# cvjena/semantic-embeddings

Hardware: AMD Instinct MI355X
Metric: retrieval_Mpairs_per_sec (higher is better)
Workload: dtype f32

## Files before the change

### semantic-embeddings_amd/csrc/rank_rows.hip

```cpp
#include "se_common.h"
#include <stdlib.h>
#include <atomic>
#include <type_traits>

namespace se {

constexpr int RK_THREADS = 512;
constexpr int RK_WAVES = RK_THREADS / WAVE;
constexpr int RK_ITEMS = 16;
constexpr int RK_TILE = RK_THREADS * RK_ITEMS;
constexpr int RK_WCHUNK = RK_TILE / RK_WAVES;
constexpr int RK_NB = 256;

struct RankLds {
    uint32_t gbase[4][RK_NB];
    uint32_t wcnt[RK_WAVES][RK_NB];
    uint32_t tile_start[RK_NB];
    uint32_t wave_tot[RK_WAVES];
    uint32_t tkeys[RK_TILE];
    uint32_t tidx[RK_TILE];
};

__device__ __forceinline__ uint32_t wave_excl_scan(uint32_t v, uint32_t &total)
{
// ... 478 lines not shown
        const int first_pad_ = ((NROW) - wave_s * (ITEMS * WAVE)) >> 6;    \
        if (first_pad_ >= ITEMS - RR_PADS) {                                                                          \
            _Pragma("unroll") for (int s = ITEMS - RR_PADS; s < ITEMS; s++) { BODY }                                  \
        } else {                                                                                                      \
            _Pragma("unroll") for (int s = 0; s < ITEMS; s++) { BODY }                                                \
        }                                                                                                             \
    }
#define RR_IDX_SCATTER_IMG(AFTER_STORE)                                                                               \
    {                                                                                                                 \
        opaque(ir[0]);                                                                                                \
        uint32_t a_ = rr_dst_mad(ir[0], xb);                                                                          \
        _Pragma("unroll") for (int s = 0; s < ITEMS; s++) {                                                           \
            uint32_t an_ = 0;                                                                                         \
            if (s + 1 < ITEMS) { opaque(ir[s + 1]); an_ = rr_dst_mad(ir[s + 1], xb); }                                \
            lds_st16_hi(a_, ir[s]);                                                                        \
            AFTER_STORE                                                                                               \
            a_ = an_;                                                                                                 \
        }                                                                                                             \
    }
    if ((int64_t)blockIdx.x < Q) {
        const float *drow = row_ptr(blockIdx.x);
        const int n0 = row_len(blockIdx.x);
        int wpos = wpos0;
        opaque(wpos);
#pragma unroll
        for (int s = 0; s < ITEMS; s++) RR_LOAD_ONE(drow, wpos, s, n0)
        if constexpr (!RAWKEYS) RR_CANON(n0)
    }
    uint32_t pf_sink = 0;
    [[maybe_unused]] int img_level = 0;
    [[maybe_unused]] bool img_again = false;
    [[maybe_unused]] int img_skip0 = 0, img_pen0 = 0, img_skip1 = 0, img_pen1 = 0;
    for (int64_t row = blockIdx.x; row < Q;) {
        const bool more = row + gridDim.x < Q;
        [[maybe_unused]] const int n_next = row_len(more ? row + gridDim.x : row);
        constexpr bool SKIP_WAVES = HWORD && ITEMS <= 88;
        const bool wave_live = !SKIP_WAVES || wave * (ITEMS * WAVE) < row_len(row);
        constexpr bool LOAD_IN_SCATTER = IMG && !SKIP_WAVES;
        bool two = false;
        [[maybe_unused]] int n_out = 0;
        if constexpr (IMG) {
            const int n_row = row_len(row);
            if (!img_again) {
                if (img_skip1 > 0) { img_level = 2; img_skip1--; }
                else if (img_skip0 > 0) { img_level = 1; img_skip0--; }
                else img_level = 0;
            }
            bool attempt = img_level < 2;
            uint32_t cbits = 0, base = 0;
            if (attempt) {
                uint32_t mb = 0;
#pragma unroll
                for (int s = 0; s + 1 < ITEMS; s += 2) mb = max(max(mb, key[s] & 0x7FFFFFFFu), key[s + 1] & 0x7FFFFFFFu);
                if constexpr (ITEMS & 1) mb = max(mb, key[ITEMS - 1] & 0x7FFFFFFFu);
#pragma unroll
                for (int off = 32; off > 0; off >>= 1) mb = max(mb, (uint32_t)__shfl_xor((int)mb, off, 64));
                if (lane == 0) wave_tot[wave] = mb;
                static_assert(!IMG || (RR_IMG_SET_WORDS == 4 * RR_THREADS && RR_IMG_SET_WORDS == RR_WIDE_WORDS && RR_IMG_SET_WORDS <= RR_IMG_WL), "one uint4 per thread, inside the worklist");
                *reinterpret_cast<uint4 *>(wlist + 4 * tid) = make_uint4(0u, 0u, 0u, 0u);
                wg_barrier();
                if (tid == 0) { ictl[0] = 0; ictl[1] = 0; }
#pragma unroll
                for (int w = 0; w < RR_WAVES; w++) mb = max(mb, wave_tot[w]);
                mb = (uint32_t)__builtin_amdgcn_readfirstlane((int)mb);
                const uint32_t e = (mb >> 23) + ((mb & 0x7FFFFFu) > 0x400000u ? 1u : 0u) - (img_level == 0 ? 1u : 0u);
                two = mb >= 0x0D800000u && mb < 0x7E800000u;
                cbits = (e + 1u) << 23;
                base = e << 23;
            }
            if (two) {
                const float c = __uint_as_float(cbits);
                int wpos_ = wpos0;
                opaque(wpos_);
                const uint32_t pk_ = ((RR_IMG_NAN_PADHI + ((uint32_t)wpos_ & 15u)) << 20) | (((uint32_t)wpos_ & 63u) << 14);
                const uint32_t tb = lds_off(tagb) + (uint32_t)wpos_;
#pragma unroll
                for (int s = 0; s < ITEMS; s++) {
                    const uint32_t t = __float_as_uint(__uint_as_float(key[s]) + c);
                    const uint32_t q = (uint32_t)rr_clamp_i32(__builtin_elementwise_sub_sat((int32_t)t, (int32_t)base), 0, 0xFEFFFF);
                    asm volatile("ds_write_b8 %0, %1 offset:%2" ::"v"(tb), "v"(q), "n"(s * WAVE) : "memory");
                    key[s] = q << 8;
                }
                if (wave_s * (ITEMS * WAVE) + ITEMS * WAVE > n_row) {
                    RR_PAD_LOOP(n_row, key[s] = (wpos_ + s * WAVE >= n_row) ? pk_ : key[s];)
                }
            } else {
                RR_CANON(n_row)
            }
            RR_T(8)
        }
        if constexpr (WIDE && VAR == 2) {
            uint32_t *stat = wave_tot;
            uint2 *outl = reinterpret_cast<uint2 *>(wcnt);
            const int n_row = row_len(row);
            int32_t mxi = 0;
            uint32_t umx = 0;
#pragma unroll
            for (int s = 0; s + 1 < ITEMS; s += 2) {
                mxi = max(max(mxi, rr_clamp_i32((int32_t)key[s], 0, 0x7F800000)), rr_clamp_i32((int32_t)key[s + 1], 0, 0x7F800000));
                umx = max(max(umx, key[s]), key[s + 1]);
            }
            if constexpr (ITEMS & 1) { mxi = max(mxi, rr_clamp_i32((int32_t)key[ITEMS - 1], 0, 0x7F800000)); umx = max(umx, key[ITEMS - 1]); }
            mxi = umx > 0xFF800000u ? 0x7F800000 : mxi;
#pragma unroll
            for (int off = 32; off > 0; off >>= 1) mxi = max(mxi, __shfl_xor(mxi, off, 64));
            if (lane == 0) stat[wave] = (uint32_t)mxi;
            if (tid == 0) stat[2 * RR_WAVES] = 0;
            RR_T(9)
            wg_barrier();
            RR_T(10)
#pragma unroll
            for (int w = 0; w < RR_WAVES; w++) mxi = max(mxi, (int32_t)stat[w]);
            const int32_t kmax = __builtin_amdgcn_readfirstlane(mxi);
            const int32_t lo = kmax > (int32_t)RR_TWO_SPAN ? kmax - (int32_t)RR_TWO_SPAN : 1, lo1 = lo - 1;
            uint32_t below_l = 0;
            {
                int wpos = wpos0;
                opaque(wpos);
#pragma unroll
                for (int s = 0; s < ITEMS; s++) below_l += ((int32_t)key[s] < lo) ? 1u : 0u;
                if (wave_s * (ITEMS * WAVE) + ITEMS * WAVE > n_row) {
                    int32_t lo_b = lo;
                    opaque(lo_b);
                    RR_PAD_LOOP(n_row, below_l -= (wpos + s * WAVE >= n_row && (int32_t)key[s] < lo_b) ? 1u : 0u;)
                }
            }
            uint32_t below_w = below_l;
#pragma unroll
            for (int off = 32; off > 0; off >>= 1) below_w += (uint32_t)__shfl_xor((int)below_w, off, 64);
            if (lane == 0) stat[RR_WAVES + wave] = below_w;
            RR_T(11)
            wg_barrier();
            uint32_t below = 0;
#pragma unroll
            for (int w = 0; w < RR_WAVES; w++) below += stat[RR_WAVES + w];
            two = kmax > 0 && below <= (uint32_t)RR_TWO_OUT;
            n_out = (int)below;
            if (two) {
                int wpos = wpos0;
                opaque(wpos);
                if (below_w != 0) {
                    int32_t lo_c = lo;
                    opaque(lo_c);
#pragma unroll
                    for (int s = 0; s < ITEMS; s++)
                        if ((int32_t)key[s] < lo_c && wpos + s * WAVE < n_row)
                            outl[atomicAdd(&stat[2 * RR_WAVES], 1u)] = make_uint2(rr_key(key[s], false, 0u), (uint32_t)(wpos + s * WAVE));
                }
#pragma unroll
                for (int s = 0; s < ITEMS; s++)
                    key[s] = (uint32_t)rr_clamp_i32(__builtin_elementwise_sub_sat((int32_t)key[s], lo1), 0, 0xFFFFFF) << 8;
                if (wave_s * (ITEMS * WAVE) + ITEMS * WAVE > n_row) {
                    RR_PAD_LOOP(n_row, key[s] = (wpos + s * WAVE >= n_row) ? 0xFFFFFF00u : key[s];)
                }
            } else {
                RR_CANON(n_row)
            }
            RR_T(8)
        }
        __builtin_amdgcn_sched_barrier(0);
        {
            int wpos = wpos0;
            opaque(wpos);
#pragma unroll
            for (int s = 0; s < ITEMS; s++) ir[s] = (uint32_t)(wpos + s * WAVE) << 16;
        }
#pragma unroll 1
        for (int p = 0; p < NPASS; p++) {
            const int shift = two ? 8 + 12 * p : (WIDE ? p * 10 : p * BITS);
            const int end = two ? (p == 1 ? 32 : 20)
                                : (WIDE ? (p == 2 ? 32 : shift + 10) : ((shift + BITS < 32) ? shift + BITS : 32));
            const bool wide = WIDE && (two || p == 2);
            uint32_t *pcnt = wcnt;
            int pcw = CNT_WORDS;
            const bool shared0 = IMG && two && p == 0;
            if (shared0) {
                pcnt = wlist;
                pcw = 0;
            } else if (wide) {
                if (!(RAWKEYS && two && p == 0)) wg_barrier();
                pcnt = reinterpret_cast<uint32_t *>(xbuf);
                pcw = RR_WIDE_WORDS;
            }
            uint32_t *mycnt = pcnt + wave * pcw;
            const uint32_t cb = lds_off(mycnt);
            auto one_set = [&]() -> bool {
                if constexpr (!IMG) return false;
                int z = pcw;
                asm volatile("" : "+s"(z));
                return z == 0;
            };
            if constexpr (IMG) {
                if (!one_set()) {
#pragma unroll
                    for (int j = 0; j < CNT_WORDS / (4 * WAVE); j++) reinterpret_cast<uint4 *>(mycnt)[j * WAVE + lane] = make_uint4(0u, 0u, 0u, 0u);
                    if (wide) {
#pragma unroll
                        for (int j = CNT_WORDS / (4 * WAVE); j < RR_WIDE_WORDS / (4 * WAVE); j++) reinterpret_cast<uint4 *>(mycnt)[j * WAVE + lane] = make_uint4(0u, 0u, 0u, 0u);
                    }
                }
            } else {
#pragma unroll
                for (int j = 0; j < CNT_WORDS / WAVE; j++) mycnt[j * WAVE + lane] = 0;
                if (wide) {
#pragma unroll
                    for (int j = CNT_WORDS / WAVE; j < RR_WIDE_WORDS / WAVE; j++) mycnt[j * WAVE + lane] = 0;
                }
            }
            [[maybe_unused]] const uint32_t wlo = wide ? 11u : 10u, whi = (uint32_t)(end - shift) - wlo, hshift = (uint32_t)(shift + (int)wlo) & 31u;
            if constexpr (HWORD) {
                if (wave_live) {
                    uint32_t hr[RR_GH], hs[RR_GH], hg[RR_GH];
                    RRRankHW<ITEMS, PEEL>::run(ir, key, hr, hs, hg, (uint32_t)shift, hshift, wlo, whi, cb, lane, end >= 32 && !two);
                }
            }
            else RRRank<ITEMS>::run(ir, key, shift, lane, cb);
            lds_wait();
            RR_T(1)
            wg_barrier();
            if constexpr (!HWORD) {
            uint32_t ex = 0;
            if (tid < RK_NB) {
                uint32_t run = 0;
#pragma unroll
                for (int w = 0; w < RR_WAVES; w++) run += wcnt[w * RK_NB + tid];
                uint32_t wtot;
                ex = wave_excl_scan(run, wtot);
                if (lane == 63) wave_tot[wave] = wtot;
            }
            wg_barrier();
            if (tid < RK_NB) {
                for (int w = 0; w < wave; w++) ex += wave_tot[w];
#pragma unroll
                for (int w = 0; w < RR_WAVES; w++) {
                    const uint32_t c = wcnt[w * RK_NB + tid];
                    wcnt[w * RK_NB + tid] = ex;
                    ex += c;
                }
            }
            } else {
                const bool scanner = tid < RR_SCAN_THREADS;
                const int st = scanner ? tid : 0;
                uint32_t T0 = 0, T1 = 0, U0 = 0, U1 = 0;
#pragma unroll
                for (int w = 0; w < RR_WAVES; w++) {
                    if (w == 1 && one_set()) break;
                    const uint2 v = *reinterpret_cast<const uint2 *>(pcnt + w * pcw + 2 * st);
                    T0 += v.x; T1 += v.y;
                }
                if (wide) {
                    __builtin_amdgcn_sched_barrier(0);
#pragma unroll
                    for (int w = 0; w < RR_WAVES; w++) {
                        if (w == 1 && one_set()) break;
                        const uint2 v = *reinterpret_cast<const uint2 *>(pcnt + w * pcw + CNT_WORDS + 2 * st);
                        U0 += v.x; U1 += v.y;
                    }
                    __builtin_amdgcn_sched_barrier(0);
                }
                uint32_t wtot, wtot2 = 0, ex2 = 0;
                uint32_t ex = wave_excl_scan(T0 + T1, wtot);
                if (wide) ex2 = wave_excl_scan(U0 + U1, wtot2);
                if (scanner && lane == 63) { wave_tot[wave] = wtot; wave_tot[RR_SCAN_WAVES + wave] = wtot2; }
                wg_barrier();
                uint32_t all = 0, all2 = 0;
#pragma unroll
                for (int w = 0; w < RR_SCAN_WAVES; w++) {
                    const uint32_t wt = wave_tot[w], wt2 = wave_tot[RR_SCAN_WAVES + w];
                    all += wt; all2 += wt2;
                    ex += (w < wave) ? wt : 0u;
                    ex2 += (w < wave) ? wt2 : 0u;
                }
                ex2 += all;
                const uint32_t hi = (all + all2) << 16;
                ex += hi; ex2 += hi;
                if (scanner) {
                uint32_t s0 = ex, s1 = ex + T0;
#pragma unroll
                for (int w = 0; w < RR_WAVES; w++) {
                    if (w == 1 && one_set()) break;
                    uint2 *wp = reinterpret_cast<uint2 *>(pcnt + w * pcw + 2 * tid);
                    const uint2 v = *wp;
                    *wp = make_uint2(s0, s1);
                    s0 += v.x; s1 += v.y;
                }
                if (wide) {
                    __builtin_amdgcn_sched_barrier(0);
                    s0 = ex2; s1 = ex2 + U0;
#pragma unroll
                    for (int w = 0; w < RR_WAVES; w++) {
                        if (w == 1 && one_set()) break;
                        uint2 *wp = reinterpret_cast<uint2 *>(pcnt + w * pcw + CNT_WORDS + 2 * tid);
                        const uint2 v = *wp;
                        *wp = make_uint2(s0, s1);
                        s0 += v.x; s1 += v.y;
                    }
                }
                }
            }
            wg_barrier();
            RR_T(2)
            if (!(IMG && two)) { RR_PREFETCH_NEXT_ROW() }
            if (wave_live) {
#pragma unroll
            for (int s0 = 0; s0 < ITEMS; s0 += 8) {
                uint32_t first[8];
#pragma unroll
                for (int g = 0; g < 8; g++)
                    if (s0 + g < ITEMS) {
                        if constexpr (HWORD) first[g] = reinterpret_cast<const uint16_t *>(mycnt)[(__builtin_amdgcn_ubfe(key[s0 + g], (uint32_t)shift, wlo) << 1) | __builtin_amdgcn_ubfe(key[s0 + g], hshift, whi)];
                        else first[g] = mycnt[(key[s0 + g] >> shift) & 0xFFu];
                    }
#pragma unroll
                for (int g = 0; g < 8; g++)
                    if (s0 + g < ITEMS) {
                        ir[s0 + g] += first[g];
                        opaque(ir[s0 + g]);
                    }
                __builtin_amdgcn_sched_barrier(0);
            }
            }
            if (wide && !one_set()) wg_barrier();
            RR_T(3)
            if constexpr (LOAD_IN_SCATTER) {
                if (end >= 32) break;
            }
            if (wave_live) {
                if constexpr (LOAD_IN_SCATTER) {
                    RR_IDX_SCATTER_IMG()
                } else {
#pragma unroll
                    for (int s = 0; s < ITEMS; s++) { opaque(ir[s]); lds_st16_hi(RR_DST(ir[s]), ir[s]); }
                }
            }
            lds_wait();
            wg_barrier();
            RR_T(4)
            const bool last = end >= 32;
            if (last) {
                if constexpr (!SEG) break;
                else {
                    RR_STREAM_PLANE(0, row)
                    wg_barrier();
                }
            } else {
                if (wave_live) rr_read_back<ITEMS, true>(ir, ring, rt, rb);
                lds_wait();
                wg_barrier();
            }
            RR_T(5)
            if (wave_live) {
#pragma unroll
                for (int s = 0; s < ITEMS; s++) { opaque(ir[s]); lds_st16_hi(RR_DST(ir[s]), key[s]); }
            }
            lds_wait();
            wg_barrier();
            if (SEG && last) {
                RR_STREAM_PLANE(1, row)
            } else {
                if (wave_live) rr_read_back<ITEMS, true>(key, ring, rt, rb);
                lds_wait();
            }
            if (end < 16 || SEG) {
                wg_barrier();
                if (wave_live) {
#pragma unroll
                    for (int s = 0; s < ITEMS; s++) { opaque(ir[s]); lds_st16_lo(RR_DST(ir[s]), key[s]); }
                }
                lds_wait();
                wg_barrier();
                if (SEG && last) break;
                if (wave_live) rr_read_back<ITEMS, false>(key, ring, rt, rb);
                lds_wait();
            }
            RR_T(6)
        }
#undef RR_DST
        if constexpr (WIDE && VAR == 2) {
            if (two && n_out > 1) {
                const uint2 *outl = reinterpret_cast<const uint2 *>(wcnt);
                if (tid < n_out) {
                    const uint2 me = outl[tid];
                    int r = 0;
                    for (int j = 0; j < n_out; j++) {
                        const uint2 o = outl[j];
                        r += (o.x < me.x || (o.x == me.x && o.y < me.y)) ? 1 : 0;
                    }
                    xbuf[r] = (uint16_t)me.y;
                }
                wg_barrier();
            }
        }
        [[maybe_unused]] bool img_fail = false;
        if constexpr (IMG) {
            const float *drow = row_ptr(more ? row + gridDim.x : row);
            int wpos = wpos0;
            opaque(wpos);
            if constexpr (LOAD_IN_SCATTER) {
                RR_IDX_SCATTER_IMG(RR_LOAD_ONE(drow, wpos, s, n_next))
                lds_wait();
                wg_barrier();
                RR_T(4)
            } else {
#pragma unroll
                for (int s = 0; s < ITEMS; s++) RR_LOAD_ONE(drow, wpos, s, n_next)
            }
        }
        if constexpr (IMG) {
            if (two) {
                int n_row = row_len(row);
                int tsc = wave_s * WAVE + (int)wave_prefix_count(~0u, ~0u);
                opaque(n_row);
                opaque(tsc);
                const float *drow_cur = row_ptr(row);
                constexpr int NS = RR_THREADS * ITEMS;
                constexpr int NG = (NS / 8 + RR_THREADS - 1) / RR_THREADS;
                uint32_t S[NG];
                uint32_t nstart = 0;
                uint4 xg[NG];
                uint32_t nxg[NG];
#pragma unroll
                for (int g = 0; g < NG; g++) {
                    const int b0 = (tsc + RR_THREADS * g) * 8;
                    const int bs = b0 < NS ? b0 : 0;
                    xg[g] = *reinterpret_cast<const uint4 *>(xbuf + bs);
                    nxg[g] = xbuf[(tsc & 63) == 63 ? (bs + 8 < NS ? bs + 8 : bs) : 0];
                }
                constexpr int TD = 1;
                uint32_t t[TD + 1][9];
                auto tag_reads = [&](int g, uint32_t (&tt)[9]) {
                    const uint32_t xi[4] = {xg[g].x, xg[g].y, xg[g].z, xg[g].w};
#pragma unroll
                    for (int j = 0; j < 4; j++) {
                        tt[2 * j] = tagb[xi[j] & 0xFFFFu];
                        tt[2 * j + 1] = tagb[xi[j] >> 16];
                    }
                    tt[8] = tagb[nxg[g]];
                };
#pragma unroll
                for (int g = 0; g < TD && g < NG; g++) tag_reads(g, t[g % (TD + 1)]);
#pragma unroll
                for (int g = 0; g < NG; g++) {
                    if (g + TD < NG) tag_reads(g + TD, t[(g + TD) % (TD + 1)]);
                    const uint32_t (&tc)[9] = t[g % (TD + 1)];
                    const bool live = (tsc + RR_THREADS * g) * 8 < n_row - 1;
                    const uint32_t A = tc[0] | (tc[1] << 8) | (tc[2] << 16) | (tc[3] << 24), B = tc[4] | (tc[5] << 8) | (tc[6] << 16) | (tc[7] << 24);
                    const uint32_t t8 = (uint32_t)__builtin_amdgcn_update_dpp((int)tc[8], (int)tc[0], 0x130, 0xF, 0xF, false);
                    const uint32_t zA = A ^ __builtin_amdgcn_alignbyte(B, A, 1), zB = B ^ __builtin_amdgcn_alignbyte(t8, B, 1);
                    const uint32_t uA = (zA & 0x7F7F7F7Fu) + 0x7F7F7F7Fu, uB = (zB & 0x7F7F7F7Fu) + 0x7F7F7F7Fu;
                    const uint32_t eA = __builtin_amdgcn_bitop3_b32(uA, zA, 0x80808080u, 0x02), eB = __builtin_amdgcn_bitop3_b32(uB, zB, 0x80808080u, 0x02);
                    S[g] = live ? ((eA >> 7) | (eB >> 3)) : 0u;
                    nstart += (uint32_t)__popc(S[g]);
                }
                uint32_t slot = 0;
                {
                    const uint32_t ca = lds_off(&ictl[0]);
                    asm volatile("ds_add_rtn_u32 %0, %1, %2\n\ts_waitcnt lgkmcnt(0)" : "=v"(slot) : "v"(ca), "v"(nstart) : "memory");
                }
#pragma unroll
                for (int g = 0; g < NG; g++) {
                    uint32_t st = S[g];
                    const int b0 = (tsc + RR_THREADS * g) * 8;
                    while (st) {
                        const int bit = __builtin_ctz(st);
                        st &= st - 1u;
                        const int pos = b0 + (bit & 4) + (bit >> 3);
                        if (slot < (uint32_t)RR_IMG_WL) wlist[slot] = pos < n_row - 1 ? (uint32_t)pos : 0xFFFFFFFFu;
                        slot++;
                    }
                }
                if constexpr (PROF) { RR_T(9) }
                wg_barrier();
                const uint32_t nwork = ictl[0];
                img_fail = nwork > (uint32_t)RR_IMG_WL;
                RR_T(11)
                if (!img_fail) {
                    constexpr int GB = 2;
#pragma unroll 1
                    for (uint32_t e0 = 0; e0 < nwork; e0 += RR_THREADS * GB) {
                        uint32_t pp[GB], im[GB], ia[GB], ib[GB], ic[GB], id[GB], tm[GB], t0[GB], t2[GB], t3[GB], ka[GB], kb[GB], kc[GB];
#pragma unroll
                        for (int k = 0; k < GB; k++) {
                            const uint32_t e = e0 + (uint32_t)(k * RR_THREADS + tsc);
                            pp[k] = e < nwork ? wlist[e] : 0xFFFFFFFFu;
                        }
#pragma unroll
                        for (int k = 0; k < GB; k++) {
                            const uint32_t p = pp[k] != 0xFFFFFFFFu ? pp[k] : 0u;
                            im[k] = xbuf[p ? p - 1u : 0u]; ia[k] = xbuf[p]; ib[k] = xbuf[p + 1];
                            ic[k] = xbuf[p + 2 < (uint32_t)NS ? p + 2 : p]; id[k] = xbuf[p + 3 < (uint32_t)NS ? p + 3 : p];
                        }
#pragma unroll
                        for (int k = 0; k < GB; k++) { tm[k] = tagb[im[k]]; t0[k] = tagb[ia[k]]; t2[k] = tagb[ic[k]]; t3[k] = tagb[id[k]]; }
#pragma unroll
                        for (int k = 0; k < GB; k++) {
                            const bool mine = pp[k] != 0xFFFFFFFFu && !(pp[k] != 0u && tm[k] == t0[k]);
                            const bool three = mine && (int)pp[k] + 2 < n_row && t2[k] == t0[k];
                            ka[k] = kb[k] = kc[k] = 0u;
                            if (mine) {
                                ka[k] = __float_as_uint(drow_cur[ia[k]]);
                                kb[k] = __float_as_uint(drow_cur[ib[k]]);
                            }
                            if (three) kc[k] = __float_as_uint(drow_cur[ic[k]]);
                        }
                        uint32_t rare = 0;
#pragma unroll
                        for (int k = 0; k < GB; k++) {
                            if (pp[k] == 0xFFFFFFFFu) continue;
                            const uint32_t p = pp[k];
                            if (p != 0u && tm[k] == t0[k]) continue;
                            const bool three = (int)p + 2 < n_row && t2[k] == t0[k];
                            const bool more4 = three && (int)p + 3 < n_row && t3[k] == t0[k];
                            const uint64_t ca = ((uint64_t)rr_key(ka[k], false, 0u) << 32) | ia[k], cb = ((uint64_t)rr_key(kb[k], false, 0u) << 32) | ib[k],
                                           cc = ((uint64_t)rr_key(kc[k], false, 0u) << 32) | ic[k];
                            if (!three) {
                                if (ca > cb) { xbuf[p] = (uint16_t)ib[k]; xbuf[p + 1] = (uint16_t)ia[k]; }
                            } else if (!more4) {
                                const uint32_t ab = ca < cb, ac = ca < cc, bc = cb < cc;
                                const uint32_t ra = 2u - ab - ac, rb = ab + 1u - bc, rc = ac + bc;
                                if (ra != 0u || rb != 1u) {
                                    xbuf[p + ra] = (uint16_t)ia[k]; xbuf[p + rb] = (uint16_t)ib[k]; xbuf[p + rc] = (uint16_t)ic[k];
                                }
                            } else rare |= 1u << k;
                        }
                        static_assert(GB == 2, "the entry is picked by one select");
#pragma unroll 1
                        for (uint32_t k = 0; k < (uint32_t)GB; k++) {
                            if (!((rare >> k) & 1u)) continue;
                            const uint32_t p = k ? pp[1] : pp[0], tg = k ? t0[1] : t0[0];
                            int len = 4;
                            while (len <= RR_IMG_RUN && (int)p + len < n_row && tagb[xbuf[p + len]] == tg) len++;
                            if (len > RR_IMG_RUN) { ictl[1] = 1u; continue; }
                            uint32_t idx[RR_IMG_RUN];
                            uint64_t kk[RR_IMG_RUN];
#pragma unroll
                            for (int j = 0; j < RR_IMG_RUN; j++) idx[j] = xbuf[p + (uint32_t)(j < len ? j : 0)];
#pragma unroll
                            for (int j = 0; j < RR_IMG_RUN; j++) kk[j] = ((uint64_t)rr_key(__float_as_uint(drow_cur[idx[j]]), false, 0u) << 32) | idx[j];
#pragma unroll
                            for (int j = 0; j < RR_IMG_RUN; j++) {
                                uint32_t r = 0;
#pragma unroll
                                for (int i = 0; i < RR_IMG_RUN; i++)
                                    if (i != j) r += (i < len && kk[i] < kk[j]) ? 1u : 0u;
                                if (j < len) xbuf[p + r] = (uint16_t)idx[j];
                            }
                        }
                    }
                    wg_barrier();
                    img_fail = ictl[1] != 0u;
                }
                RR_T(10)
            }
        }
        if (!IMG || img_fail) {
            const float *drow = row_ptr((IMG && img_fail) ? row : (more ? row + gridDim.x : row));
            int wpos = wpos0;
            opaque(wpos);
#pragma unroll
            for (int s = 0; s < ITEMS; s++) RR_LOAD_ONE(drow, wpos, s, n_next)
        }
        if constexpr (IMG) {
#pragma unroll
            for (int s = 0; s < ITEMS; s++) opaque(key[s]);
            asm volatile("s_waitcnt vmcnt(0)" : "+v"(pf_sink) : : "memory");
        }
        int wt = tid;
        opaque(wt);
        const bool write_out = !IMG || !img_fail;
        if constexpr (SEG) {
            RR_STREAM_PLANE(2, row)
        } else if (!write_out) {
        } else if (idx64 == 2) {
            uint16_t *o = (uint16_t *)rank + row * ldr;
            _Pragma("unroll 2") for (int j = wt * 8; j < N; j += RR_THREADS * 8) {
                if (vec_ok && j + 7 < N) {
                    const rr_i32x4 v = *reinterpret_cast<const rr_i32x4 *>(xbuf + j);
                    __builtin_nontemporal_store(v, reinterpret_cast<rr_i32x4 *>(o + j));
                } else {
                    for (int e = 0; e < 8 && j + e < N; e++) o[j + e] = xbuf[j + e];
                }
            }
        } else if (idx64) {
            int64_t *o = (int64_t *)rank + row * ldr;
            uint2 nv = *reinterpret_cast<const uint2 *>(xbuf + (wt * 4 < N ? wt * 4 : 0));
            _Pragma("unroll 1") for (int j = wt * 4; j < N; j += RR_THREADS * 4) {
                const uint2 v = nv;
                const int jn = j + RR_THREADS * 4;
                nv = *reinterpret_cast<const uint2 *>(xbuf + (jn < N ? jn : 0));
                const int64_t e0 = v.x & 0xFFFFu, e1 = v.x >> 16, e2 = v.y & 0xFFFFu, e3 = v.y >> 16;
                if (vec_ok && j + 3 < N) {
                    __builtin_nontemporal_store((rr_i64x2){e0, e1}, reinterpret_cast<rr_i64x2 *>(o + j));
                    __builtin_nontemporal_store((rr_i64x2){e2, e3}, reinterpret_cast<rr_i64x2 *>(o + j + 2));
                } else {
                    o[j] = e0;
                    if (j + 1 < N) o[j + 1] = e1;
                    if (j + 2 < N) o[j + 2] = e2;
                    if (j + 3 < N) o[j + 3] = e3;
                }
            }
        } else {
            int32_t *o = (int32_t *)rank + row * ldr;
            constexpr int RR_WO = 4;
            _Pragma("unroll 1") for (int j0 = wt * 4; j0 < N; j0 += RR_THREADS * 4 * RR_WO) {
                uint2 v[RR_WO];
#pragma unroll
                for (int u = 0; u < RR_WO; u++) {
                    const int j = j0 + u * RR_THREADS * 4;
                    v[u] = *reinterpret_cast<const uint2 *>(xbuf + (j < N ? j : 0));
                }
#pragma unroll
                for (int u = 0; u < RR_WO; u++) {
                    const int j = j0 + u * RR_THREADS * 4;
                    if (j >= N) break;
                    const int e0 = v[u].x & 0xFFFFu, e1 = v[u].x >> 16, e2 = v[u].y & 0xFFFFu, e3 = v[u].y >> 16;
                    if (vec_ok && j + 3 < N) {
                        __builtin_nontemporal_store((rr_i32x4){e0, e1, e2, e3}, reinterpret_cast<rr_i32x4 *>(o + j));
                    } else {
                        o[j] = e0;
                        if (j + 1 < N) o[j + 1] = e1;
                        if (j + 2 < N) o[j + 2] = e2;
                        if (j + 3 < N) o[j + 3] = e3;
                    }
                }
            }
        }
        RR_T(7)
        if constexpr (!RAWKEYS) RR_CANON(n_next)
        if constexpr (PROF) {
            _Pragma("unroll") for (int s = 0; s < ITEMS; s++) opaque(key[s]);
        }
        if constexpr (!IMG)
            asm volatile("s_waitcnt vmcnt(0)" : "+v"(pf_sink) : : "memory");
        RR_T(0)
        if constexpr (IMG) {
            if (img_fail) {
                if (img_level == 0) { img_pen0 = img_pen0 ? (img_pen0 < 16 ? 2 * img_pen0 : 32) : 1; img_skip0 = img_pen0; }
                else { img_pen1 = img_pen1 ? (img_pen1 < 16 ? 2 * img_pen1 : 32) : 1; img_skip1 = img_pen1; }
                img_level++;
                img_again = true;
            } else {
                if (two) { if (img_level == 0) img_pen0 = 0; else img_pen1 = 0; }
                img_again = false;
                row += gridDim.x;
            }
        } else row += gridDim.x;
    }
    if (PROF && tid == 0)
    {
        for (int i = 0; i < 12; i++) atomicAdd(&prof[i], (unsigned long long)t_acc[i]);
    }
#undef RR_T
}

}

using namespace se;

static size_t rank_idx_bytes(int idx) { return idx == 2 ? 2 : (idx ? 8 : 4); }

static int rank_grid(int64_t q)
{
    const int64_t g = 512;
    return (int)(q < g ? q : g);
}

static int64_t rank_npad(int64_t n) { return (n + 63) / 64 * 64; }

static bool rank_use_tiled(int64_t n)
{
    static const bool force = tuning_env("SE_RANK_TILED") != nullptr;
    return force || n > RR_MAX_N;
}

__global__ __launch_bounds__(256) void rank_skew_detect_kernel(const float *__restrict__ pdist, int64_t ldp, int64_t Q, int N,
                                                               int shift, int two_ok, uint32_t *__restrict__ flag)
{
    constexpr int NBIN = 4096;
    __shared__ uint32_t hist[NBIN], hash_hist[NBIN];
    __shared__ uint32_t best, row_max[3], row_below[3], repeats;
    for (int i = threadIdx.x; i < NBIN; i += 256) { hist[i] = 0; hash_hist[i] = 0; }
    if (threadIdx.x == 0) { best = 0; repeats = 0; }
    if (threadIdx.x < 3) { row_max[threadIdx.x] = 0; row_below[threadIdx.x] = 0; }
    wg_barrier();
    const int cols = N < 1024 ? N : 1024;
    uint32_t kk[3][4];
#pragma unroll
    for (int r = 0; r < 3; r++) {
        const int64_t row = (r == 0) ? 0 : (r == 1 ? Q / 2 : Q - 1);
        const float *drow = pdist + row * ldp;
#pragma unroll
        for (int u = 0; u < 4; u++) {
            const int i = threadIdx.x + 256 * u;
            kk[r][u] = canon_key(drow[(int64_t)(i < cols ? i : 0) * N / cols]);
        }
    }
#pragma unroll
    for (int r = 0; r < 3; r++) {
#pragma unroll
        for (int u = 0; u < 4; u++) {
            const int i = threadIdx.x + 256 * u;
            if (i >= cols) continue;
            const uint32_t k = kk[r][u];
            atomicAdd(&hist[k >> shift], 1u);
            if (k != 0xFFFFFFFFu) atomicMax(&row_max[r], k);
            if (i < 256 && atomicAdd(&hash_hist[((k ^ ((uint32_t)r * 0x3C6EF372u)) * 2654435761u) >> 20], 1u) != 0u) atomicAdd(&repeats, 1u);
        }
    }
    wg_barrier();
#pragma unroll
    for (int r = 0; r < 3; r++) {
        const uint32_t lo = row_max[r] > RR_TWO_SPAN ? row_max[r] - RR_TWO_SPAN : 0u;
#pragma unroll
        for (int u = 0; u < 4; u++)
            if (threadIdx.x + 256 * u < cols && kk[r][u] < lo) atomicAdd(&row_below[r], 1u);
    }
    uint32_t mine = 0;
    for (int i = threadIdx.x; i < NBIN; i += 256) mine = hist[i] > mine ? hist[i] : mine;
    atomicMax(&best, mine);
    wg_barrier();
    if (threadIdx.x == 0) {
        const bool two = (two_ok & 1) && row_below[0] <= 4 && row_below[1] <= 4 && row_below[2] <= 4;
        const bool skewed = 10u * best >= 3u * 3u * (uint32_t)cols;
        const bool distinct = repeats < 3u * 96u;
        *flag = (two && distinct) ? 2u : (skewed ? 1u : (((two_ok & 2) && distinct) ? 3u : 0u));
    }
}

struct Resident { hipError_t err; int64_t grid; };
static Resident rank_resident(const void *kern, size_t lds)
{
    hipError_t e = hipFuncSetAttribute(kern, hipFuncAttributeMaxDynamicSharedMemorySize, (int)lds);
    int dev = 0, occ = 0;
    hipDeviceProp_t prop;
    if (e == hipSuccess) e = hipGetDevice(&dev);
    if (e == hipSuccess) e = hipGetDeviceProperties(&prop, dev);
    if (e == hipSuccess) e = hipOccupancyMaxActiveBlocksPerMultiprocessor(&occ, kern, RR_THREADS, lds);
    if (e != hipSuccess) return {e, 0};
    return {hipSuccess, (int64_t)(prop.multiProcessorCount > 0 ? prop.multiProcessorCount : 256) * (occ > 0 ? occ : 1)};
}

template <int ITEMS, bool HW, int VAR>
static int launch_rank_reg_variant(const float *pdist, int64_t ldp, int64_t q, int n, void *rank, int idx64, int64_t ldr,
                                   const uint32_t *skew_flag, hipStream_t s)
{
    const size_t lds = rr_region0_bytes<ITEMS, HW, VAR>() + 32 * sizeof(uint32_t) + (size_t)RR_THREADS * ITEMS * sizeof(uint16_t);
    static_assert(rr_region0_bytes<ITEMS, HW, VAR>() + 32 * sizeof(uint32_t) + (size_t)RR_THREADS * ITEMS * sizeof(uint16_t) <= 160 * 1024, "LDS of one CU");
    static const bool profile = tuning_env("SE_RR_PROFILE") != nullptr;
    auto kern = (kTuning && profile) ? rank_rows_reg_kernel<ITEMS, kTuning && (ITEMS == 98), HW, VAR> : rank_rows_reg_kernel<ITEMS, false, HW, VAR>;
    static const Resident res = rank_resident((const void *)kern, lds);
    if (res.err != hipSuccess) return fail(SE_ERR_HIP, "se_rank_rows: kernel set-up failed: %s", hipGetErrorString(res.err));
    int64_t grid = res.grid;
    if (grid > q) grid = q;
    const size_t esz = rank_idx_bytes(idx64);
    const int vec_ok = ((((uintptr_t)rank) & 15) == 0) && ((ldr * esz) % 16 == 0);
    unsigned long long *prof = nullptr;
    if (profile && ITEMS == 98) {
        SE_HIP_CHECK(hipMalloc((void **)&prof, 36 * sizeof(unsigned long long)));
        SE_HIP_CHECK(hipMemsetAsync(prof, 0, 36 * sizeof(unsigned long long), s));
    }
    hipLaunchKernelGGL(kern, dim3((unsigned)grid), dim3(RR_THREADS), lds, s, pdist, ldp, q, n, rank, ldr, idx64, vec_ok, prof, skew_flag, RankSeg{0, 0, nullptr, 0});
    SE_LAUNCH_CHECK();
    if (prof) {
        unsigned long long h[36];
        SE_HIP_CHECK(hipStreamSynchronize(s));
        SE_HIP_CHECK(hipMemcpy(h, prof, sizeof(h), hipMemcpyDeviceToHost));
        SE_HIP_CHECK(hipFree(prof));
        static const char *names[12] = {"load", "rank", "scan", "dest", "idx-write", "idx-read", "key-exchange", "write-out", "image-map|window-map", "tag-scan|window-max", "repair|window-barrier-1", "window-count|scan-barrier"};
        double tot = 0;
        for (int i = 0; i < 12; i++) tot += (double)h[i];
        if (tot > 0) {
            fprintf(stderr, "[se_rank_rows profile] ITEMS=%d hw=%d peel=%d grid=%lld:", ITEMS, (int)HW, VAR, (long long)grid);
            for (int i = 0; i < 12; i++) fprintf(stderr, " %s %.1f%%", names[i], 100.0 * (double)h[i] / tot);
            fprintf(stderr, "  (%.0f cycles per row; wave 0 of every workgroup, timestamps behind the phases' own barriers)", tot / (double)q);
            fprintf(stderr, "\n");
        }
    }
    return SE_OK;
}

template <int ITEMS>
static int launch_rank_reg(const float *pdist, int64_t ldp, int64_t q, int n, void *rank, int idx64, int64_t ldr, bool hw, void *scratch,
                           hipStream_t s)
{
    if (!hw) return launch_rank_reg_variant<ITEMS, false, 0>(pdist, ldp, q, n, rank, idx64, ldr, nullptr, s);
    constexpr bool wide = (size_t)RR_THREADS * ITEMS * sizeof(uint16_t) >= (size_t)RR_WAVES * RR_WIDE_WORDS * sizeof(uint32_t);
    constexpr bool two_ok = wide;
    constexpr bool img_ok = wide && ITEMS <= RR_IMG_MAX_ITEMS;
    static const char *force = tuning_env("SE_RANK_PEEL");
    if (force || !scratch) {
        if (force && force[0] == '1') return launch_rank_reg_variant<ITEMS, true, 1>(pdist, ldp, q, n, rank, idx64, ldr, nullptr, s);
        if (force && force[0] == '2' && two_ok) return launch_rank_reg_variant<ITEMS, true, two_ok ? 2 : 0>(pdist, ldp, q, n, rank, idx64, ldr, nullptr, s);
        if (force && force[0] == '3' && img_ok) return launch_rank_reg_variant<ITEMS, true, img_ok ? 3 : 0>(pdist, ldp, q, n, rank, idx64, ldr, nullptr, s);
        return launch_rank_reg_variant<ITEMS, true, 0>(pdist, ldp, q, n, rank, idx64, ldr, nullptr, s);
    }
    uint32_t *flag = (uint32_t *)scratch + 16;
    const int top_shift = wide ? 20 : 2 * RR_HW_BITS;
    hipLaunchKernelGGL(rank_skew_detect_kernel, dim3(1), dim3(256), 0, s, pdist, ldp, q, n, top_shift, (two_ok ? 1 : 0) | (img_ok ? 2 : 0), flag);
    SE_LAUNCH_CHECK();
    int rc = launch_rank_reg_variant<ITEMS, true, 0>(pdist, ldp, q, n, rank, idx64, ldr, flag, s);
    if (rc != SE_OK) return rc;
    rc = launch_rank_reg_variant<ITEMS, true, 1>(pdist, ldp, q, n, rank, idx64, ldr, flag, s);
    if (rc != SE_OK) return rc;
    if (two_ok) rc = launch_rank_reg_variant<ITEMS, true, two_ok ? 2 : 0>(pdist, ldp, q, n, rank, idx64, ldr, flag, s);
    if (rc != SE_OK || !img_ok) return rc;
    return launch_rank_reg_variant<ITEMS, true, img_ok ? 3 : 0>(pdist, ldp, q, n, rank, idx64, ldr, flag, s);
}

constexpr int RC_CAP = 1022;
constexpr int MG_THREADS = 256;
constexpr int MG_VT = 16;
constexpr int RUNS_MAX_SEG = 8;

struct MergeLevel {
    int run_n, N, pairs, tiles, tile;
    const uint16_t *planes; int64_t plane_elems; int cap;
    const uint32_t *in_key, *in_idx; int64_t ld;
};

template <bool PLANES>
__device__ __forceinline__ uint32_t level_key(const MergeLevel &L, int64_t r, int run, int i)
{
    if constexpr (PLANES) {
        const uint16_t *khi = L.planes + L.plane_elems + (r * (2 * L.pairs) + run) * (int64_t)L.cap, *klo = khi + L.plane_elems;
        return ((uint32_t)khi[i] << 16) | klo[i];
    } else return L.in_key[r * L.ld + (int64_t)run * L.run_n + i];
}
__device__ __forceinline__ int level_run_len(const MergeLevel &L, int run)
{
    const int64_t rest = (int64_t)L.N - (int64_t)run * L.run_n;
    return rest <= 0 ? 0 : (rest < L.run_n ? (int)rest : L.run_n);
}

template <bool PLANES>
__global__ __launch_bounds__(256) void rank_merge_partition_kernel(const MergeLevel L, int64_t rows, int32_t *__restrict__ splits)
{
    const int64_t g = (int64_t)blockIdx.x * 256 + threadIdx.x;
    if (g >= rows * L.pairs * (L.tiles + 1)) return;
    const int64_t rp = g / (L.tiles + 1);
    const int t = (int)(g - rp * (L.tiles + 1));
    const int64_t r = rp / L.pairs;
    const int p = (int)(rp - r * L.pairs);
    const int na = level_run_len(L, 2 * p), nb = level_run_len(L, 2 * p + 1);
    const int64_t d64 = (int64_t)t * L.tile;
    const int d = (int)(d64 < na + nb ? d64 : na + nb);
    int lo = d > nb ? d - nb : 0, hi = d < na ? d : na;
    while (lo < hi) {
        const int mid = (lo + hi) >> 1;
        if (level_key<PLANES>(L, r, 2 * p, mid) <= level_key<PLANES>(L, r, 2 * p + 1, d - 1 - mid)) lo = mid + 1;
        else hi = mid;
    }
    splits[g] = lo;
}

template <bool PLANES, typename IT>
__device__ __forceinline__ void merge_stage(const MergeLevel &L, int64_t r, int run, int e0, int cnt, uint32_t *sK, IT *sI, int dst, int tid)
{
    if constexpr (PLANES) {
        const uint16_t *ix = L.planes + (r * (2 * L.pairs) + run) * (int64_t)L.cap, *khi = ix + L.plane_elems, *klo = khi + L.plane_elems;
        const int e1 = e0 + cnt;
        for (int j = (e0 & ~3) + tid * 4; j < e1; j += MG_THREADS * 4) {
            const uint2 x = *reinterpret_cast<const uint2 *>(ix + j), h = *reinterpret_cast<const uint2 *>(khi + j), l = *reinterpret_cast<const uint2 *>(klo + j);
            const uint32_t k[4] = {(h.x << 16) | (l.x & 0xFFFFu), (h.x & 0xFFFF0000u) | (l.x >> 16), (h.y << 16) | (l.y & 0xFFFFu), (h.y & 0xFFFF0000u) | (l.y >> 16)};
            const uint32_t id[4] = {x.x & 0xFFFFu, x.x >> 16, x.y & 0xFFFFu, x.y >> 16};
#pragma unroll
            for (int e = 0; e < 4; e++) {
                const int pos = j + e - e0;
                if (pos >= 0 && pos < cnt) { sK[dst + pos] = k[e]; sI[dst + pos] = (IT)id[e]; }
            }
        }
    } else {
        const uint32_t *k = L.in_key + r * L.ld + (int64_t)run * L.run_n + e0, *ix = L.in_idx + r * L.ld + (int64_t)run * L.run_n + e0;
        for (int j = tid; j < cnt; j += MG_THREADS) { sK[dst + j] = k[j]; sI[dst + j] = (IT)ix[j]; }
    }
}

template <bool PLANES, bool OUT_RANKS, bool IDX64, int VT>
__global__ __launch_bounds__(MG_THREADS) void rank_merge_kernel(const MergeLevel L, const int32_t *__restrict__ splits, void *__restrict__ rank, int64_t ldr,
                                                                int vec_ok, uint32_t *__restrict__ out_key, uint32_t *__restrict__ out_idx)
{
    constexpr int TILE = MG_THREADS * VT;
    using IT = typename std::conditional<PLANES, uint16_t, uint32_t>::type;
    __shared__ __attribute__((aligned(16))) uint32_t sK[TILE + 8];
    __shared__ __attribute__((aligned(16))) IT sI[TILE + 8];
    const int tid = threadIdx.x;
    const int p = blockIdx.x / L.tiles, t = blockIdx.x - p * L.tiles;
    const int64_t r = blockIdx.y;
    const int na_run = level_run_len(L, 2 * p), nb_run = level_run_len(L, 2 * p + 1);
    const int64_t o0 = (int64_t)t * TILE;
    if (o0 >= na_run + nb_run) return;
    const int32_t *sp = splits + (r * L.pairs + p) * (int64_t)(L.tiles + 1) + t;
    const int a0 = sp[0], a1 = sp[1];
    const int tot = (int)((o0 + TILE < na_run + nb_run ? o0 + TILE : na_run + nb_run) - o0);
    const int b0 = (int)o0 - a0;
    const int na = a1 - a0, nb = tot - na;
    merge_stage<PLANES>(L, r, 2 * p, a0, na, sK, sI, 0, tid);
    merge_stage<PLANES>(L, r, 2 * p + 1, b0, nb, sK, sI, na, tid);
    wg_barrier();
    const int d = tid * VT < tot ? tid * VT : tot;
    int lo = d > nb ? d - nb : 0, hi = d < na ? d : na;
    while (lo < hi) {
        const int mid = (lo + hi) >> 1;
        if (sK[mid] <= sK[na + d - 1 - mid]) lo = mid + 1;
        else hi = mid;
    }
    int a = lo, b = d - lo;
    uint32_t ka = a < na ? sK[a] : 0u, kb = b < nb ? sK[na + b] : 0u;
    const uint32_t base_a = PLANES ? (uint32_t)(2 * p) * (uint32_t)L.run_n : 0u, base_b = PLANES ? base_a + (uint32_t)L.run_n : 0u;
    uint32_t out[VT];
    [[maybe_unused]] uint32_t outk[OUT_RANKS ? 1 : VT];
#pragma unroll
    for (int i = 0; i < VT; i++) {
        const bool take_a = (b >= nb) || (a < na && ka <= kb);
        const int pp = take_a ? a : na + b;
        out[i] = (uint32_t)sI[pp < tot ? pp : 0] + (take_a ? base_a : base_b);
        if constexpr (!OUT_RANKS) outk[i] = take_a ? ka : kb;
        if (take_a) { a++; ka = sK[a < na ? a : 0]; }
        else { b++; kb = sK[na + (b < nb ? b : 0)]; }
    }
    wg_barrier();
    if constexpr (OUT_RANKS) {
#pragma unroll
        for (int i = 0; i < VT; i++) sK[tid * VT + i] = out[i];
        wg_barrier();
        if constexpr (IDX64) {
            int64_t *o = (int64_t *)rank + r * ldr + o0;
            for (int j = tid * 2; j < tot; j += MG_THREADS * 2) {
                if (vec_ok && j + 1 < tot) *reinterpret_cast<longlong2 *>(o + j) = make_longlong2((int64_t)sK[j], (int64_t)sK[j + 1]);
                else { o[j] = sK[j]; if (j + 1 < tot) o[j + 1] = sK[j + 1]; }
            }
        } else {
            int32_t *o = (int32_t *)rank + r * ldr + o0;
            for (int j = tid * 4; j < tot; j += MG_THREADS * 4) {
                if (vec_ok && j + 3 < tot) *reinterpret_cast<uint4 *>(o + j) = *reinterpret_cast<const uint4 *>(sK + j);
                else
                    for (int e = 0; e < 4 && j + e < tot; e++) o[j + e] = (int32_t)sK[j + e];
            }
        }
    } else {
        const int64_t ob = r * L.ld + (int64_t)(2 * p) * L.run_n + o0;
#pragma unroll
        for (int i = 0; i < VT; i++) sK[tid * VT + i] = outk[i];
        wg_barrier();
        for (int j = tid; j < tot; j += MG_THREADS) out_key[ob + j] = sK[j];
        wg_barrier();
#pragma unroll
        for (int i = 0; i < VT; i++) sK[tid * VT + i] = out[i];
        wg_barrier();
        for (int j = tid; j < tot; j += MG_THREADS) out_idx[ob + j] = sK[j];
    }
}

static int rank_merge_vt()
{
    if (kTuning) { const char *e = tuning_env("SE_MG_VT"); if (e) { const int v = atoi(e); if (v == 8 || v == 12 || v == 24) return v; } }
    return MG_VT;
}

static int rank_runs_segments(int64_t n)
{
    static const bool off = tuning_env("SE_RANK_NORUNS") != nullptr;
    if (off || n <= RR_MAX_N) return 0;
    for (int sgm = 2; sgm <= RUNS_MAX_SEG; sgm *= 2)
        if (((n + sgm - 1) / sgm + 7) / 8 * 8 <= RR_MAX_N) return sgm;
    return 0;
}
static bool rank_runs_ok(int64_t n) { return rank_runs_segments(n) != 0; }
static int64_t rank_runs_seg_n(int64_t n) { const int sgm = rank_runs_segments(n); return ((n + sgm - 1) / sgm + 7) / 8 * 8; }
static int rank_runs_items(int64_t n)
{
    const int items = (int)((rank_runs_seg_n(n) + RR_THREADS - 1) / RR_THREADS);
    return items <= 64 ? 64 : items <= 72 ? 72 : items <= 80 ? 80 : items <= 88 ? 88 : items <= 98 ? 98 : 104;
}
constexpr int64_t RUNS_HEAD = 256 + 4 * (RC_CAP + 2);
struct RunsLayout { int64_t chunk, cap, tile, split_words, head, split_bytes, plane_bytes, level_bytes, total; int sgm; };
static RunsLayout rank_runs_layout(int64_t q, int64_t n)
{
    RunsLayout y;
    y.sgm = rank_runs_segments(n);
    y.cap = (int64_t)RR_THREADS * rank_runs_items(n);
    y.tile = (int64_t)MG_THREADS * rank_merge_vt();
    const int64_t per_row = 6 * y.sgm * y.cap + (y.sgm > 2 ? 8 * (n + 8) : 0) + (y.sgm > 4 ? 8 * (n + 8) : 0);
    int64_t c = (int64_t)3072 * 1024 * 1024 / per_row;
    c = c > 4096 ? 4096 : (c < 64 ? 64 : c);
    if (kTuning) { const char *e = tuning_env("SE_RANK_CHUNK"); if (e && atoll(e) > 0) c = atoll(e); }
    y.chunk = q < c ? q : c;
    const int64_t seg_n = rank_runs_seg_n(n);
    int64_t most = 0;
    for (int64_t pairs = y.sgm / 2, run = seg_n; pairs >= 1; pairs /= 2, run *= 2) {
        const int64_t words = y.chunk * pairs * ((2 * run + y.tile - 1) / y.tile + 1);
        most = words > most ? words : most;
    }
    y.split_words = most;
    y.head = (RUNS_HEAD + 255) / 256 * 256;
    y.split_bytes = (most * 4 + 255) / 256 * 256;
    y.plane_bytes = (3 * y.sgm * y.chunk * y.cap * 2 + 255) / 256 * 256;
    y.level_bytes = y.sgm > 2 ? (y.chunk * (n + 8) * 4 + 255) / 256 * 256 : 0;
    y.total = y.head + y.split_bytes + y.plane_bytes + (y.sgm > 2 ? 2 : 0) * y.level_bytes + (y.sgm > 4 ? 2 : 0) * y.level_bytes;
    return y;
}
static int64_t rank_runs_bytes(int64_t q, int64_t n) { return rank_runs_layout(q, n).total; }

template <bool PLANES, bool OUT_RANKS>
static int launch_merge_level(const MergeLevel &L, int64_t rows, int32_t *splits, void *rout, int idx64, int64_t ldr, int vec_ok, uint32_t *out_key,
                              uint32_t *out_idx, int vt, hipStream_t s)
{
    const int64_t nsplit = rows * L.pairs * (L.tiles + 1);
    hipLaunchKernelGGL(rank_merge_partition_kernel<PLANES>, dim3((unsigned)((nsplit + 255) / 256)), dim3(256), 0, s, L, rows, splits);
    SE_LAUNCH_CHECK();
    const dim3 mgrid((unsigned)(L.pairs * L.tiles), (unsigned)rows);
#define SE_MG_LAUNCH(I64, V) hipLaunchKernelGGL((rank_merge_kernel<PLANES, OUT_RANKS, I64, V>), mgrid, dim3(MG_THREADS), 0, s, L, splits, rout, ldr, vec_ok, out_key, out_idx)
    if (kTuning && vt != MG_VT) {
        if (vt == 8) { if (OUT_RANKS && idx64) SE_MG_LAUNCH(true, 8); else SE_MG_LAUNCH(false, 8); }
        else if (vt == 12) { if (OUT_RANKS && idx64) SE_MG_LAUNCH(true, 12); else SE_MG_LAUNCH(false, 12); }
        else { if (OUT_RANKS && idx64) SE_MG_LAUNCH(true, 24); else SE_MG_LAUNCH(false, 24); }
    } else if (OUT_RANKS && idx64) SE_MG_LAUNCH(true, MG_VT);
    else SE_MG_LAUNCH(false, MG_VT);
#undef SE_MG_LAUNCH
    SE_LAUNCH_CHECK();
    return SE_OK;
}

// ... 434 lines not shown
```

Baseline: 244,000.

## Pipeline count lookups and replace per-lane LDS atomics with wave reductions

The per-item count lookup loop becomes a software pipeline with a lag of up to eight items, so loads for later items overlap the adds for earlier ones instead of running in batches of eight. The work-list slot allocation now does one wave-level inclusive scan and a single ds_add from lane 63, instead of one LDS atomic per lane. The small sampling/classification kernel replaces per-thread LDS atomicMax/atomicAdd on shared counters with wave shuffle reductions followed by one atomic per wave. These changes aim to reduce LDS atomic contention and latency stalls, at the cost of extra cross-lane shuffles and inline asm that assumes a 64-lane wave.

Measured after the change: 245,500 (median of 6 runs). Within noise of the previous version (+0.6%).

```diff
diff --git a/semantic-embeddings_amd/csrc/rank_rows.hip b/semantic-embeddings_amd/csrc/rank_rows.hip
--- a/semantic-embeddings_amd/csrc/rank_rows.hip
+++ b/semantic-embeddings_amd/csrc/rank_rows.hip
@@ -804,23 +804,20 @@
             RR_T(2)
             if (!(IMG && two)) { RR_PREFETCH_NEXT_ROW() }
             if (wave_live) {
-#pragma unroll
-            for (int s0 = 0; s0 < ITEMS; s0 += 8) {
-                uint32_t first[8];
-#pragma unroll
-                for (int g = 0; g < 8; g++)
-                    if (s0 + g < ITEMS) {
-                        if constexpr (HWORD) first[g] = reinterpret_cast<const uint16_t *>(mycnt)[(__builtin_amdgcn_ubfe(key[s0 + g], (uint32_t)shift, wlo) << 1) | __builtin_amdgcn_ubfe(key[s0 + g], hshift, whi)];
-                        else first[g] = mycnt[(key[s0 + g] >> shift) & 0xFFu];
+                constexpr int RR_GD = ITEMS < 8 ? ITEMS : 8;
+                uint32_t first[RR_GD];
+#pragma unroll
+                for (int s = 0; s < ITEMS + RR_GD; s++) {
+                    if (s >= RR_GD) {
+                        ir[s - RR_GD] += first[s % RR_GD];
+                        opaque(ir[s - RR_GD]);
                     }
-#pragma unroll
-                for (int g = 0; g < 8; g++)
-                    if (s0 + g < ITEMS) {
-                        ir[s0 + g] += first[g];
-                        opaque(ir[s0 + g]);
+                    if (s < ITEMS) {
+                        if constexpr (HWORD) first[s % RR_GD] = reinterpret_cast<const uint16_t *>(mycnt)[(__builtin_amdgcn_ubfe(key[s], (uint32_t)shift, wlo) << 1) | __builtin_amdgcn_ubfe(key[s], hshift, whi)];
+                        else first[s % RR_GD] = mycnt[(key[s] >> shift) & 0xFFu];
                     }
-                __builtin_amdgcn_sched_barrier(0);
-            }
+                    __builtin_amdgcn_sched_barrier(0);
+                }
             }
             if (wide && !one_set()) wg_barrier();
             RR_T(3)
@@ -957,7 +954,14 @@
                 uint32_t slot = 0;
                 {
                     const uint32_t ca = lds_off(&ictl[0]);
-                    asm volatile("ds_add_rtn_u32 %0, %1, %2\n\ts_waitcnt lgkmcnt(0)" : "=v"(slot) : "v"(ca), "v"(nstart) : "memory");
+                    const uint32_t incl = wave_incl_scan(nstart);
+                    uint32_t got = 0;
+                    uint64_t saved;
+                    asm volatile("s_and_saveexec_b64 %0, %4\n\tds_add_rtn_u32 %1, %2, %3\n\ts_waitcnt lgkmcnt(0)\n\ts_mov_b64 exec, %0"
+                                 : "=&s"(saved), "+v"(got)
+                                 : "v"(ca), "v"(incl), "s"(1ull << 63)
+                                 : "memory");
+                    slot = (uint32_t)__builtin_amdgcn_readlane((int)got, 63) + (incl - nstart);
                 }
 #pragma unroll
                 for (int g = 0; g < NG; g++) {
@@ -1197,29 +1201,45 @@
             kk[r][u] = canon_key(drow[(int64_t)(i < cols ? i : 0) * N / cols]);
         }
     }
+    const bool lead = (threadIdx.x & 63) == 0;
+    auto wave_umax = [](uint32_t v) -> uint32_t {
+#pragma unroll
+        for (int off = 32; off > 0; off >>= 1) v = max(v, (uint32_t)__shfl_xor((int)v, off, 64));
+        return (uint32_t)__builtin_amdgcn_readfirstlane((int)v);
+    };
+    auto wave_usum = [](uint32_t v) -> uint32_t { return (uint32_t)__builtin_amdgcn_readfirstlane(wave_sum((int)v)); };
+    uint32_t rep = 0;
 #pragma unroll
     for (int r = 0; r < 3; r++) {
+        uint32_t mx = 0;
 #pragma unroll
         for (int u = 0; u < 4; u++) {
             const int i = threadIdx.x + 256 * u;
             if (i >= cols) continue;
             const uint32_t k = kk[r][u];
             atomicAdd(&hist[k >> shift], 1u);
-            if (k != 0xFFFFFFFFu) atomicMax(&row_max[r], k);
-            if (i < 256 && atomicAdd(&hash_hist[((k ^ ((uint32_t)r * 0x3C6EF372u)) * 2654435761u) >> 20], 1u) != 0u) atomicAdd(&repeats, 1u);
-        }
-    }
+            if (k != 0xFFFFFFFFu) mx = max(mx, k);
+            if (i < 256 && atomicAdd(&hash_hist[((k ^ ((uint32_t)r * 0x3C6EF372u)) * 2654435761u) >> 20], 1u) != 0u) rep++;
+        }
+        mx = wave_umax(mx);
+        if (lead) atomicMax(&row_max[r], mx);
+    }
+    rep = wave_usum(rep);
+    if (lead) atomicAdd(&repeats, rep);
     wg_barrier();
 #pragma unroll
     for (int r = 0; r < 3; r++) {
         const uint32_t lo = row_max[r] > RR_TWO_SPAN ? row_max[r] - RR_TWO_SPAN : 0u;
-#pragma unroll
-        for (int u = 0; u < 4; u++)
-            if (threadIdx.x + 256 * u < cols && kk[r][u] < lo) atomicAdd(&row_below[r], 1u);
+        uint32_t below = 0;
+#pragma unroll
+        for (int u = 0; u < 4; u++) below += ((int)threadIdx.x + 256 * u < cols && kk[r][u] < lo) ? 1u : 0u;
+        below = wave_usum(below);
+        if (lead) atomicAdd(&row_below[r], below);
     }
     uint32_t mine = 0;
     for (int i = threadIdx.x; i < NBIN; i += 256) mine = hist[i] > mine ? hist[i] : mine;
-    atomicMax(&best, mine);
+    mine = wave_umax(mine);
+    if (lead) atomicMax(&best, mine);
     wg_barrier();
     if (threadIdx.x == 0) {
         const bool two = (two_ok & 1) && row_below[0] <= 4 && row_below[1] <= 4 && row_below[2] <= 4;
```
